# faustomorales/keras-ocr

Measured on AMD Instinct MI355X. Metric: images/sec end-to-end Pipeline.recognize() @768x768, higher is better.
Workload: dtype f32 (fp32 operands as 2 fp16 pieces [F(4,3) / head layers] or 3 bf16 pieces [1x1, dilated], 3 / 6 MFMA products, fp32 accumulate; fp32-class error vs fp64: tests/test_conv_gpu.py)

## Files before the change

keras_ocr_amd/csrc/api.cpp:

```cpp
#include "abi.h"
#include "taps.h"
#include <cmath>
#include <algorithm>
#include <mutex>
#include <set>

int arena_reserve(kocr_ctx* ctx, Arena& a, size_t bytes) {
  ctx->invalidate_results();
  a.requested = bytes;
  a.peak = 0;
  const size_t guard = a.gctx ? ARENA_GUARD_RESERVE : 0;
  if (bytes + guard <= a.cap) return KOCR_OK;
  if (a.base) {
    if (!a.guards.empty()) arena_guard_check(a);
    KOCR_HIP(ctx, hipStreamSynchronize(ctx->stream));
    KOCR_HIP(ctx, hipFree(a.base));
    a.base = nullptr;
    a.cap = 0;
  }
  const size_t want = bytes + (bytes >> 3) + 4096 + guard;
  void* p = nullptr;
  hipError_t e = hipMalloc(&p, want);
  if (e != hipSuccess) {
    ctx->set_err("workspace hipMalloc(" + std::to_string(want) + " B) failed: " + hipGetErrorString(e));
// ... 267 lines not shown
  TapsEnd taps_end{ctx, TAPS_CRNN};
  return crnn_batches(ctx, M, batch);
}

extern "C" {

int kocr_create(kocr_ctx** out, int hip_device) {
  if (!out) return KOCR_EINVAL;
  *out = nullptr;
  int count = 0;
  if (hipGetDeviceCount(&count) != hipSuccess || hip_device < 0 || hip_device >= count) return KOCR_EHIP;
  if (hipSetDevice(hip_device) != hipSuccess) return KOCR_EHIP;
  kocr_ctx* c = new kocr_ctx();
  if (const char* e = getenv("KOCR_SPLIT"))
    c->split_mode = (!strcmp(e, "f16") || !strcmp(e, "fp16") || !strcmp(e, "f16x2")) ? KOCR_SPLIT_F16X2
                    : (!strcmp(e, "f16x1") || !strcmp(e, "fast"))                     ? KOCR_SPLIT_F16X1
                                                                                      : KOCR_SPLIT_BF16X3;
  {
    auto on = [](const char* name, bool dflt) {
      const char* e = getenv(name);
      return e ? atoi(e) != 0 : dflt;
    };
    c->sw.dense_splitk = on("KOCR_DENSE_SPLITK", true);
    c->sw.lstm16 = on("KOCR_LSTM16", true);
    c->sw.hs16 = on("KOCR_HS16", true);
    c->sw.k5 = on("KOCR_K5", true);
    c->sw.up2x = on("KOCR_UP2X", true);
    c->sw.w43h = on("KOCR_W43H", true);
    c->sw.w43 = on("KOCR_W43", true);
    c->sw.w43r = on("KOCR_W43R", true);
    c->sw.w43v = on("KOCR_W43V", true);
    c->sw.w43rag = on("KOCR_W43RAG", true);
    c->sw.w43dilh = on("KOCR_W43DILH", true);
    c->sw.cells = on("KOCR_CELLS", true);
    c->sw.wsplit = on("KOCR_WSPLIT", true);
    c->sw.dsplit = on("KOCR_DSPLIT", true);
    c->sw.hsplit = on("KOCR_HSPLIT", true);
    c->sw.first = on("KOCR_FIRST", true);
  }
  c->prof_layers = getenv("KOCR_PROF_LAYERS") != nullptr;
  if (const char* e = getenv("KOCR_LINFOLD")) c->opt_linfold = atoi(e) != 0;
  if (const char* e = getenv("KOCR_UPFOLD")) c->opt_upfold = atoi(e) != 0;
  c->device = hip_device;
  if (hipDeviceGetAttribute(&c->n_cu, hipDeviceAttributeMultiprocessorCount, hip_device) != hipSuccess ||
      hipStreamCreateWithFlags(&c->own_stream, hipStreamNonBlocking) != hipSuccess) {
    delete c;
    return KOCR_EHIP;
  }
  c->stream = c->own_stream;
  *out = c;
  return KOCR_OK;
}

void kocr_destroy(kocr_ctx* ctx) {
  if (!ctx) return;
  hipSetDevice(ctx->device);
  hipStreamSynchronize(ctx->stream);
  craft_free(ctx);
  crnn_free(ctx);
  for (void* p : ctx->owned) hipFree(p);
  for (Arena* a : {&ctx->ws, &ctx->pp, &ctx->pp2, &ctx->io, &ctx->pl, &ctx->bx, &ctx->chw, &ctx->chr})
    if (a->base) hipFree(a->base);
  for (auto& pd : ctx->pending) {
    hipEventDestroy(pd.a);
    hipEventDestroy(pd.b);
  }
// ... 1145 lines not shown
```

keras_ocr_amd/csrc/common.h:

```cpp
#pragma once
#include <hip/hip_runtime.h>
#include <stdint.h>
#include <string>
#include <vector>
#include <map>
#include <atomic>
#include <cstdio>
#include <cstring>
#include <type_traits>
#include "../../include/kocr.h"

#define KOCR_HIP(ctx, expr)                                                         \
  do {                                                                              \
    hipError_t _e = (expr);                                                         \
    if (_e != hipSuccess) {                                                         \
      (ctx)->set_err(std::string(#expr) + ": " + hipGetErrorString(_e) + " at " +   \
                     __FILE__ + ":" + std::to_string(__LINE__));                    \
      return KOCR_EHIP;                                                             \
    }                                                                               \
  } while (0)

#define KOCR_TRY(expr)            \
  do {                            \
    int _rc = (expr);             \
// ... 113 lines not shown
    return c;
  }
};

struct PatternTables {
  const int* hdr = nullptr;
  const int2* nodes = nullptr;
  const int2* states = nullptr;
  const int* pred = nullptr;
};

struct kocr_ctx {
  int device = 0;
  hipStream_t own_stream = nullptr;
  hipStream_t stream = nullptr;
  std::string err;
  void set_err(const std::string& s) { err = s; }

  int split_mode = KOCR_SPLIT_F16X2;
  bool opt_linfold = true, opt_upfold = true;
  int min_area_rect = KOCR_RECT_EXACT;
  struct Switches {
    bool dense_splitk = true;
    bool lstm16 = true;
    bool hs16 = true;
    bool k5 = true;
    bool up2x = true;
    bool w43h = true;
    bool w43 = true;
    bool w43r = true;
    bool w43v = true;
    bool w43rag = true;
    bool w43dilh = true;
    bool cells = true;
    bool wsplit = true;
    bool dsplit = true;
    bool hsplit = true;
    bool first = true;
  } sw;
  bool prof_layers = false;
  int n_cu = 0;

  unsigned* d_amax = nullptr;
  int amax_used = 0;
  static constexpr int AMAX_SLOTS = 1 << 16;
  int amax_begin();
  unsigned* amax_slots(int n);

  Arena ws, pp, pp2, io, pl;
  Arena bx;
  static constexpr int N_ARENAS = 8;
  inline Arena* arena_at(int i);
  static const char* arena_name(int i) {
    static const char* const names[N_ARENAS] = {"ws", "pp", "pp2", "io", "pl", "bx", "chw", "chr"};
    return i >= 0 && i < N_ARENAS ? names[i] : nullptr;
  }
  struct GuardDamage {
    int count = 0, arena = -1;
    size_t offset = 0, byte = 0;
  } guard_damage;
  int ws_reserve(size_t bytes);
  void ws_reset() { ws.reset(); }
  void* ws_alloc(size_t bytes);

  std::vector<void*> owned;
  int dev_alloc(void** out, size_t bytes);
// ... 510 lines not shown
```

keras_ocr_amd/csrc/conv_w43.hip:

```cpp
#include "w43_common.h"
#include <utility>


template <int POOL, int DBG = 0, int DIL = 0>
__global__ __launch_bounds__(256) void conv_w43_kernel(W4Params p) {
  extern __shared__ __attribute__((aligned(16))) unsigned short As[];
  const int tid = threadIdx.x, lane = tid & 63;
  const int wn = __builtin_amdgcn_readfirstlane(tid >> 6);
  const int l31 = lane & 31, l5 = lane >> 5;
  const int nblk_n = p.Cout_pad >> 7;
  const int total = p.total_tiles;
  const int ns = p.nsteps;
  const int G = gridDim.x;
  constexpr unsigned OOB = 0x80000000u;

  const int qi = tid >> 2, q4 = tid & 3;
  const int ldst = ((qi >> 5) * 2 + (q4 >> 1)) * KH_STRIDE + ((((qi & 31) * 8) ^ ((q4 >> 1) * 32)) + (q4 & 1) * 4);
  struct Geo {
    unsigned goff[6];
    int gy;
    bool gok;
    const float* base;
  };
  auto make_geo = [&](int L, Geo& g) __attribute__((always_inline)) {
// ... 599 lines not shown
  extern __shared__ __attribute__((aligned(16))) unsigned short As[];
  const int tid = threadIdx.x, lane = tid & 63;
  const int wave = __builtin_amdgcn_readfirstlane(tid >> 6);
  const int wn = wave & 1, ph = wave >> 1;
  const int l31 = lane & 31, l5 = lane >> 5;
  const int total = p.total_tiles;
  const int ncg = p.Cin >> 4;
  const int G = gridDim.x;
  constexpr unsigned OOB = 0x80000000u;

  auto tile_mt = [&](int mp, int m) {
    if constexpr (GEO) {
      const int rq = (int)w4_fdiv((unsigned)mp, p.dv_tpr), cb = mp - rq * p.tiles_per_row;
      return (2 * rq + m) * p.tiles_per_row + cb;
    } else {
      return 2 * mp + m;
    }
  };

  const int q4 = tid & 3, qd0 = (tid >> 2) & (QPR - 1), r0 = GEO ? (tid >> 6) : (tid >> 7);
  const int cp = tid & 7, qd1 = GEO ? ((tid >> 3) & 15) : qd0, r1 = GEO ? 4 + (tid >> 7) : r0 + 2;
  int ldst[2];
  ldst[0] = r0 * ROW_STRIDE + (q4 >> 1) * KHS + (((qd0 * 8) ^ ((q4 >> 1) * 32)) + (q4 & 1) * 4);
  if constexpr (GEO)
    ldst[1] = r1 * ROW_STRIDE + (cp >> 2) * KHS + (((qd1 * 8) ^ ((cp >> 2) * 32)) + (cp & 3) * 2);
  else
    ldst[1] = r1 * ROW_STRIDE + (q4 >> 1) * KHS + (((qd1 * 8) ^ ((q4 >> 1) * 32)) + (q4 & 1) * 4);
  struct Geo {
    unsigned off0[2];
    unsigned ok;
    const float* base;
  };
  auto make_geo = [&](int L, Geo& g, bool& left, bool& right) __attribute__((always_inline)) {
    const int mp = kocr_xcd_remap(L < total ? L : 0, total);
    int y0, x0;
    const long pm = w4_mtile_pm0<1>(p, tile_mt(mp, 0), y0, x0);
    g.base = p.in + (pm * p.in_cs + p.in_co) - (long)(p.W + 1) * p.in_cs;
    g.off0[0] = (unsigned)(((r0 * p.W + 4 * qd0) * p.in_cs + q4 * 4) * 4);
    g.off0[1] = (unsigned)(((r1 * p.W + 4 * qd1) * p.in_cs + (GEO ? cp * 2 : q4 * 4)) * 4);
    g.ok = ((L < total && (unsigned)(y0 - 1 + r0) < (unsigned)p.H) ? 1u : 0u) |
           ((L < total && (unsigned)(y0 - 1 + r1) < (unsigned)p.H) ? 2u : 0u);
    left = x0 == 0;
    right = x0 + TCOLS >= p.W;
  };
  Geo gc, gn;
  bool lc, rc, ln, rn;
  int ld_cg = 0;
  bool ld_next = false;
  typedef typename std::conditional<GEO != 0, v2f, v4f>::type raw1_t;
  auto load_item0 = [&](v4f (&raw)[6]) __attribute__((always_inline)) {
    const int soff = ld_cg * 64;
    const bool ok = (ld_next ? gn.ok : gc.ok) & 1u;
    const unsigned off0 = (ld_next ? gn.off0[0] : gc.off0[0]) | (ok ? 0u : OOB);
    const bool left = (ld_next ? ln : lc) && qd0 == 0, right = (ld_next ? rn : rc) && qd0 == QPR - 1;
    const unsigned stride = (unsigned)(p.in_cs * 4);
    const __amdgpu_buffer_rsrc_t rsrc = w4_rsrc(ld_next ? gn.base : gc.base, 0x80000000u);
#pragma unroll
    for (int k = 0; k < 6; ++k) {
      const unsigned padk = (k == 0 ? (left ? OOB : 0u) : 0u) | (k == 5 ? (right ? OOB : 0u) : 0u);
      raw[k] = __builtin_bit_cast(v4f, __builtin_amdgcn_raw_buffer_load_b128(rsrc, (off0 + k * stride) | padk, soff, 0));
    }
  };
  auto load_item1 = [&](raw1_t (&raw)[6]) __attribute__((always_inline)) {
    const int soff = ld_cg * 64;
    const bool ok = ((ld_next ? gn.ok : gc.ok) >> 1) & 1u;
    const unsigned off0 = (ld_next ? gn.off0[1] : gc.off0[1]) | (ok ? 0u : OOB);
    const bool left = (ld_next ? ln : lc) && qd1 == 0, right = (ld_next ? rn : rc) && qd1 == QPR - 1;
// ... 91 lines not shown
        mfma12(cur, pp);
      }
      __builtin_amdgcn_sched_barrier(0);
      {
        int sn = s0 + ky + 1;
        sn = sn >= ns ? sn - ns : sn;
        w4_load_w(bw[pp], w_ptr + (size_t)sn * w_step, 3 * ph + pp);
      }
      if (g == 3) load_item0(raw0);
    }
    load_item1(raw1);
    advance();
  };

  make_geo(blockIdx.x, gc, lc, rc);
  make_geo(blockIdx.x + G, gn, ln, rn);
  load_item0(raw0);
  load_item1(raw1);
  advance();
#pragma unroll
  for (int pl = 0; pl < 3; ++pl) w4_load_w(bw[pl], w_ptr, 3 * ph + pl);
#pragma unroll
  for (int xi = 0; xi < 6; ++xi) {
    produce4(raw0, As, xi, 0);
    produce_item1(As, xi);
  }
  load_item0(raw0);
  load_item1(raw1);
  advance();
  __syncthreads();
  load_a(a0, As, 0, 0);

  for (int L = blockIdx.x; L < total; L += G) {
    const int mp = kocr_xcd_remap(L, total);
#pragma unroll
    for (int x = 0; x < 3; ++x)
#pragma unroll
      for (int m = 0; m < 2; ++m)
#pragma unroll
        for (int r = 0; r < 16; ++r) acc[x][m][r] = 0.f;
    __builtin_amdgcn_s_waitcnt(0x0F70);
    for (int cg = 0; cg < ncg; cg += 2) {
      phase(As, As + BUF_R, 3 * cg, 0);
      phase(As + BUF_R, As, 3 * cg + 3, 1);
    }
    gc = gn;
    lc = ln;
    rc = rn;
    make_geo(L + 2 * G, gn, ln, rn);
    ld_next = false;

    {
      const int n = wn * 32 + l31;
      const int nc = n < p.Cout ? n : p.Cout - 1;
      const float pa = p.pre_a[nc], pb = p.pre_b[nc];
      const bool has_post = p.post_a != nullptr;
      const float qa = has_post ? p.post_a[nc] : 1.f, qb = has_post ? p.post_b[nc] : 0.f;
      const bool live = n < p.Cout;
      const float lo = p.relu ? 0.f : -INFINITY;
      auto act = [&](float v) { return fmaxf(v * pa + pb, lo); };
      v4f* xch = reinterpret_cast<v4f*>(As + BUF_R);
      float out[4][16];
      auto halves = [&](auto ph_c) __attribute__((always_inline)) {
        constexpr int PH = decltype(ph_c)::value;
        auto partial = [&](auto m_c, int r, float (&o)[4]) __attribute__((always_inline)) {
          constexpr int M = decltype(m_c)::value;
          const float u = acc[0][M][r], v = acc[1][M][r], w = acc[2][M][r];
// ... 113 lines not shown
    if constexpr (GEO == 2)
      return ((w >> 1) * 2 + kh) * 128 + (w & 1) * 64 + ((q * 8) ^ (kh * 32));
    else
      return w * ROW_STRIDE + kh * KHS + ((q * 8) ^ (kh * 32));
  };
  auto tile_org = [&](int mp, int& y0, int& x0) -> long {
    if constexpr (GEO == 2) {
      const int rq = (int)w4_fdiv((unsigned)mp, p.dv_tpr), cb = mp - rq * p.tiles_per_row;
      const int ho = p.H >> 3;
      const int nimg = (int)w4_fdiv((unsigned)rq, p.dv_hh), ro = rq - nimg * ho;
      y0 = 8 * ro;
      x0 = 32 * cb;
      return ((long)nimg * p.H + y0) * p.W + x0;
    } else {
      const int rq = (int)w4_fdiv((unsigned)mp, p.dv_tpr), cb = mp - rq * p.tiles_per_row;
      return w4_mtile_pm0<1>(p, 2 * rq * p.tiles_per_row + cb, y0, x0);
    }
  };

  const int q4 = tid & 3, qd0 = (tid >> 2) & (QPR - 1), r0 = GEO == 2 ? (tid >> 5) : (tid >> 6);
  const int cp = tid & 7;
  const int qd1 = GEO == 2 ? ((tid >> 3) & 7) : ((tid >> 3) & 15);
  const int r1 = GEO == 2 ? 8 + ((tid >> 6) & 1) : 4 + (tid >> 7);
  int ldst[2];
  ldst[0] = slot(r0, q4 >> 1, qd0) + (q4 & 1) * 4;
  ldst[1] = slot(r1, cp >> 2, qd1) + (cp & 3) * 2;
  struct Geo {
    unsigned off0[2];
    unsigned ok;
    const float* base;
  };
  auto make_geo = [&](int L, Geo& g, bool& left, bool& right) __attribute__((always_inline)) {
    int mp, nt_unused;
    w4_decode(p, kocr_xcd_remap(L < total ? L : 0, total), nblk_n, mp, nt_unused);
    int y0, x0;
    const long pm = tile_org(mp, y0, x0);
    g.base = p.in + (pm * p.in_cs + p.in_co) - (long)(p.W + 1) * p.in_cs;
    g.off0[0] = (unsigned)(((r0 * p.W + 4 * qd0) * p.in_cs + q4 * 4) * 4);
    g.off0[1] = (unsigned)(((r1 * p.W + 4 * qd1) * p.in_cs + cp * 2) * 4);
    g.ok = ((L < total && (unsigned)(y0 - 1 + r0) < (unsigned)p.H) ? 1u : 0u) |
           ((L < total && (unsigned)(y0 - 1 + r1) < (unsigned)p.H) ? 2u : 0u);
    left = x0 == 0;
    right = x0 + TCOLS >= p.W;
  };
  Geo gc, gn;
  bool lc, rc, ln, rn;
  int ld_cg = 0;
  bool ld_next = false;
  auto load_item0 = [&](v4f (&raw)[6]) __attribute__((always_inline)) {
    const int soff = ld_cg * 64;
    const bool ok = (ld_next ? gn.ok : gc.ok) & 1u;
    const unsigned off0 = (ld_next ? gn.off0[0] : gc.off0[0]) | (ok ? 0u : OOB);
    const bool left = (ld_next ? ln : lc) && qd0 == 0, right = (ld_next ? rn : rc) && qd0 == QPR - 1;
    const unsigned stride = (unsigned)(p.in_cs * 4);
    const __amdgpu_buffer_rsrc_t rsrc = w4_rsrc(ld_next ? gn.base : gc.base, 0x80000000u);
#pragma unroll
    for (int k = 0; k < 6; ++k) {
      const unsigned padk = (k == 0 ? (left ? OOB : 0u) : 0u) | (k == 5 ? (right ? OOB : 0u) : 0u);
      raw[k] = __builtin_bit_cast(v4f, __builtin_amdgcn_raw_buffer_load_b128(rsrc, (off0 + k * stride) | padk, soff, 0));
    }
  };
  auto load_item1 = [&](v2f (&raw)[6]) __attribute__((always_inline)) {
    const int soff = ld_cg * 64;
    const bool ok = ((ld_next ? gn.ok : gc.ok) >> 1) & 1u;
    const unsigned off0 = (ld_next ? gn.off0[1] : gc.off0[1]) | (ok ? 0u : OOB);
    const bool left = (ld_next ? ln : lc) && qd1 == 0, right = (ld_next ? rn : rc) && qd1 == QPR - 1;
    const unsigned stride = (unsigned)(p.in_cs * 4);
// ... 81 lines not shown
      mfma12(a0, 2 * q);
      interleave();
      __builtin_amdgcn_sched_barrier(0);
      load_b(2 * q);
      __builtin_amdgcn_sched_barrier(0);
      if (q < 2) {
        load_a(a0, bufc, KY, 2 * q + 2);
        produce(2 * q + 1);
        mfma12(a1, 2 * q + 1);
        interleave();
      } else if constexpr (KY < 2) {
        load_a(a0, bufc, KY + 1, 0);
        produce(5);
        mfma12(a1, 5);
        interleave();
      } else {
        __syncthreads();
        load_a(a0, bufn, 0, 0);
        __builtin_amdgcn_sched_barrier(0);
        mfma12(a1, 5);
      }
      __builtin_amdgcn_sched_barrier(0);
      load_b(2 * q + 1);
    }
  };

  make_geo(blockIdx.x, gc, lc, rc);
  make_geo(blockIdx.x + G, gn, ln, rn);
  load_item0(raw0);
  load_item1(raw1);
  advance();
  {
    int mp0, nt0;
    w4_decode(p, kocr_xcd_remap(blockIdx.x, total), nblk_n, mp0, nt0);
    const unsigned short* w0 = w_tile(nt0);
#pragma unroll
    for (int xi = 0; xi < 6; ++xi) w4_load_w(bw[xi], w0, xi);
  }
#pragma unroll
  for (int xi = 0; xi < 6; ++xi) {
    produce4(raw0, As, xi, 0);
    produce_item1(As, xi);
  }
  load_item0(raw0);
  load_item1(raw1);
  advance();
  __syncthreads();
  load_a(a0, As, 0, 0);

  for (int L = blockIdx.x; L < total; L += G) {
    int mp, nt, mp_n, nt_n;
    w4_decode(p, kocr_xcd_remap(L, total), nblk_n, mp, nt);
    w4_decode(p, kocr_xcd_remap(L + G < total ? L + G : L, total), nblk_n, mp_n, nt_n);
    const unsigned short* w_ptr = w_tile(nt);
    const unsigned short* w_after = w_tile(nt_n);
    auto w_at = [&](int s) { return s < ns ? w_ptr + (size_t)s * w_step : w_after; };
#pragma unroll
    for (int x = 0; x < 6; ++x)
#pragma unroll
      for (int m = 0; m < 2; ++m)
#pragma unroll
        for (int r = 0; r < 16; ++r) acc[x][m][r] = 0.f;
    __builtin_amdgcn_s_waitcnt(0x0F70);
    for (int cg = 0; cg < ncg; cg += 2) {
      step(std::integral_constant<int, 0>{}, As, As + BUF_R, w_at(3 * cg + 1));
      load_item0(raw0);
      step(std::integral_constant<int, 1>{}, As, As + BUF_R, w_at(3 * cg + 2));
      load_item1(raw1);
      advance();
      step(std::integral_constant<int, 2>{}, As, As + BUF_R, w_at(3 * cg + 3));
      step(std::integral_constant<int, 0>{}, As + BUF_R, As, w_at(3 * cg + 4));
      load_item0(raw0);
      step(std::integral_constant<int, 1>{}, As + BUF_R, As, w_at(3 * cg + 5));
      load_item1(raw1);
      advance();
      step(std::integral_constant<int, 2>{}, As + BUF_R, As, w_at(3 * cg + 6));
    }
    gc = gn;
    lc = ln;
    rc = rn;
    make_geo(L + 2 * G, gn, ln, rn);
    ld_next = false;

    {
      const int n = (nt * 4 + wn) * 32 + l31;
      const int nc = n < p.Cout ? n : p.Cout - 1;
// ... 316 lines not shown
      p.cellWv = in.cellWv;
      p.cells_per_row = in.W / in.cellW;
    }
  }
  w4_div_magic((unsigned)(p.qpr > 0 ? p.qpr : 1), p.dv_qpr);
  w4_div_magic((unsigned)L.dil, p.dv_dil);
  w4_div_magic((unsigned)in.H, p.dv_h);
  w4_div_magic((unsigned)(p.rq_per_img ? p.rq_per_img : 1), p.dv_rq);
  w4_div_magic((unsigned)(p.cellW ? p.cellW : 1), p.dv_wc);
  p.total_tiles = p.n_mpairs * (p.Cout_pad / (narrow ? 64 : 128));
  w4_div_magic((unsigned)p.tiles_per_row, p.dv_tpr);
  w4_div_magic((unsigned)(geo2 ? in.H / 8 : in.H / 2), p.dv_hh);
  w4_div_magic((unsigned)p.n_mpairs, p.dv_mp);
  w4_div_magic((unsigned)(in.H * in.W), p.dv_hw);
  if (q.tracks()) {
    p.amax_out = (!fuse || need_full) ? out.amax : nullptr;
    p.amax_pool = fuse ? pool->amax : nullptr;
  }
  if (q.pieces) {
    const unsigned* slots = in.amax;
    if (!slots) {
      unsigned* tmp = ctx->amax_slots(in.N);
      if (!tmp) KOCR_FAIL(ctx, KOCR_ECAPACITY, "conv " + L.name + ": out of max-|x| slots");
      KOCR_TRY(launch_absmax(ctx, in, tmp));
      slots = tmp;
    }
    p.amax_in = slots;
    if (ctx->range_on) KOCR_TRY(launch_range_stats(ctx, L.name, in, slots, 12));
    p.wgt = L.d_w4h;
    p.pre_a = L.d_pre_a_h;
  }
  w4_div_magic((unsigned)(p.Cout_pad / (narrow ? 64 : 128)), p.dv_nb);
  p.m_fastest = (size_t)L.Cin * L.w4_cout_pad * 3 * 36 > ((size_t)6 << 20) ? 1 : 0;
  std::string nm, fam;
  w43_names(ctx, L, q, nm, fam);
  kocr_note_dispatch(fam.c_str(), L, in);
  const double Malg = cells ? (double)in.N * in.cells() * (in.H - 1) * in.cellWv : (double)M;
  const double flops = 2.0 * Malg * L.Kreal * L.Cout;
  const double bytes = 4.0 * (Malg * L.Cin + Malg * L.Cout * ((fuse && !need_full) ? 0.25 : 1.0) + (double)L.Kreal * L.Cout);
  {
    ProfScope ps(ctx, nm.c_str(), flops, bytes);
#ifdef KOCR_DEV_SWITCHES
    static const int dbg = getenv("KOCR_W43_DBG") ? atoi(getenv("KOCR_W43_DBG")) : 0;
    if (dbg >= 1 && dbg <= 15 && !fuse) return w4_launch_dbg(ctx, p, dbg, std::make_integer_sequence<int, 15>{});
#endif
    switch (q.arr) {
      case 'v':
        if (q.pieces)
          KOCR_TRY(launch_w43vh(ctx, p, fuse, q.geo, q.pieces, q.mode));
        else if (q.geo == 2)
          KOCR_TRY((w4v_launch<0, 2>(ctx, p)));
        else
          KOCR_TRY((fuse ? w4v_launch<1, 1>(ctx, p) : w4v_launch<0, 1>(ctx, p)));
        break;
      case 'r':
        if (q.pieces)
          KOCR_TRY(launch_w43rh(ctx, p, fuse, q.pieces, q.mode));
        else if (q.geo == 1)
          KOCR_TRY((fuse ? w4r_launch<1, 1>(ctx, p) : w4r_launch<0, 1>(ctx, p)));
        else
          KOCR_TRY((fuse ? w4r_launch<1, 0>(ctx, p) : w4r_launch<0, 0>(ctx, p)));
        break;
      case 'f': KOCR_TRY(launch_w43fh(ctx, p, q.pieces)); break;
      case 'n': KOCR_TRY(fuse ? w4n_launch<1>(ctx, p) : w4n_launch<0>(ctx, p)); break;
      default:
        if (L.dil != 1)
// ... 13 lines not shown
```

keras_ocr_amd/csrc/conv_w43h.hip:

```cpp
#include "w43_common.h"
#include "probe_clock.h"

namespace {

#define W4H_SCALED_CONSTANTS(sc)                                                                       \
  const float k_s = (sc), k_sA = (sc) * W4_A, k_sB = (sc) * W4_B, k_sA2 = (sc) * W4_A2, k_sB2 = (sc) * W4_B2, \
              k_sA2B2 = (sc) * W4_A2B2, k_sA2PB2 = (sc) * W4_A2PB2
template <class T>
__device__ __forceinline__ T w4h_transform(const T (&d)[6], int xi, float k_s, float k_sA, float k_sB, float k_sA2, float k_sB2,
                                           float k_sA2B2, float k_sA2PB2) {
  switch (xi) {
    case 0: return (k_sA2B2 * d[0] - k_sA2PB2 * d[2]) + k_s * d[4];
    case 1: return (k_s * d[4] - k_sB2 * d[2]) + k_sA * (d[3] - W4_B2 * d[1]);
    case 2: return (k_s * d[4] - k_sB2 * d[2]) - k_sA * (d[3] - W4_B2 * d[1]);
    case 3: return (k_s * d[4] - k_sA2 * d[2]) + k_sB * (d[3] - W4_A2 * d[1]);
    case 4: return (k_s * d[4] - k_sA2 * d[2]) - k_sB * (d[3] - W4_A2 * d[1]);
    default: return (k_sA2B2 * d[1] - k_sA2PB2 * d[3]) + k_s * d[5];
  }
}

constexpr int W4H_TOP = 12;

}

// ... 37 lines not shown
      y0 = (GEO == 2 ? 8 : 4) * ro;
      x0 = TCOLS * cb;
      nimg_o = nimg;
      return ((long)nimg * p.H + y0) * p.W + x0;
    } else if constexpr (GEO == 2) {
      const int rq = (int)w4_fdiv((unsigned)mp, p.dv_tpr), cb = mp - rq * p.tiles_per_row;
      const int ho = p.H >> 3;
      const int nimg = (int)w4_fdiv((unsigned)rq, p.dv_hh), ro = rq - nimg * ho;
      y0 = 8 * ro;
      x0 = 32 * cb;
      return ((long)nimg * p.H + y0) * p.W + x0;
    } else {
      const int rq = (int)w4_fdiv((unsigned)mp, p.dv_tpr), cb = mp - rq * p.tiles_per_row;
      return w4_mtile_pm0<1>(p, 2 * rq * p.tiles_per_row + cb, y0, x0);
    }
  };

  const int q4 = tid & 3, qd0 = (tid >> 2) & (QPR - 1), r0 = GEO == 2 ? (tid >> 5) : (tid >> 6);
  const int cp = tid & 7;
  const int qd1 = GEO == 2 ? ((tid >> 3) & 7) : ((tid >> 3) & 15);
  const int r1 = GEO == 2 ? 8 + ((tid >> 6) & 1) : 4 + (tid >> 7);
  int ldst[2];
  ldst[0] = slot(r0, q4 >> 1, qd0) + (q4 & 1) * 4;
  ldst[1] = slot(r1, cp >> 2, qd1) + (cp & 3) * 2;
  struct Geo {
    unsigned off0[2];
    unsigned ok;
    int e;
    int e1, qb;
    const float* base;
  };
  auto make_geo = [&](int L, Geo& g, bool& left, bool& right) __attribute__((always_inline)) {
    int mp, nt_unused;
    w4_decode(p, kocr_xcd_remap(L < total ? L : 0, total), nblk_n, mp, nt_unused);
    int y0, x0, nimg = 0;
    const long pm = tile_org(mp, y0, x0, nimg);
    g.base = p.in + (pm * p.in_cs + p.in_co) - (long)(p.W + 1) * p.in_cs;
    const int tid = wn * 64 + kocr_fresh_lane();
    const int q4 = tid & 3, qd0 = (tid >> 2) & (QPR - 1), r0 = GEO == 2 ? (tid >> 5) : (tid >> 6);
    const int cp = tid & 7;
    const int qd1 = GEO == 2 ? ((tid >> 3) & 7) : ((tid >> 3) & 15);
    const int r1 = GEO == 2 ? 8 + ((tid >> 6) & 1) : 4 + (tid >> 7);
    g.off0[0] = (unsigned)(((r0 * p.W + 4 * qd0) * p.in_cs + q4 * 4) * 4);
    g.off0[1] = (unsigned)(((r1 * p.W + 4 * qd1) * p.in_cs + cp * 2) * 4);
    g.ok = ((L < total && (unsigned)(y0 - 1 + r0) < (unsigned)p.H) ? 1u : 0u) |
           ((L < total && (unsigned)(y0 - 1 + r1) < (unsigned)p.H) ? 2u : 0u);
    g.e1 = 0;
    g.qb = QPR;
    if constexpr (MODE == 2) {
      const int j0 = (int)w4_fdiv((unsigned)x0, p.dv_wc);
      const int j1 = j0 + 1 < p.cells_per_row ? j0 + 1 : j0;
      const int c0 = __builtin_amdgcn_readfirstlane(nimg * p.cells_per_row + j0), c1 = __builtin_amdgcn_readfirstlane(nimg * p.cells_per_row + j1);
      g.e = kocr_scale_exp_bits(kocr_sload(p.amax_in + c0), W4H_TOP);
      g.e1 = kocr_scale_exp_bits(kocr_sload(p.amax_in + c1), W4H_TOP);
      const int qb = ((j0 + 1) * p.cellW - x0) >> 2;
      g.qb = qb < QPR ? qb : QPR;
    } else if constexpr (MODE == 1) {
      g.e = kocr_scale_exp_bits(kocr_sload(p.amax_in + __builtin_amdgcn_readfirstlane(nimg)), W4H_TOP);
    } else {
      g.e = kocr_scale_exp_bits(kocr_sload(p.amax_in + __builtin_amdgcn_readfirstlane((int)w4_fdiv((unsigned)pm, p.dv_hw))), W4H_TOP);
    }
    if constexpr (MODE == 1) {
      const int c0 = x0 - 1 + 4 * qd0, c1 = x0 - 1 + 4 * qd1;
      unsigned cm = 0;
#pragma unroll
      for (int k = 0; k < 6; ++k)
        cm |= ((unsigned)(c0 + k) < (unsigned)p.W ? 0u : (4u << k)) | ((unsigned)(c1 + k) < (unsigned)p.W ? 0u : (256u << k));
// ... 190 lines not shown
      interleave();
      __builtin_amdgcn_sched_barrier(0);
      load_b(2 * q);
      __builtin_amdgcn_sched_barrier(0);
      if (q < 2) {
        load_a(a0, bufc, KY, 2 * q + 2);
        produce(2 * q + 1);
        mfma_pt(a1, bw[SLOT][2 * q + 1], 2 * q + 1);
        interleave();
      } else if constexpr (KY < 2) {
        load_a(a0, bufc, KY + 1, 0);
        produce(5);
        mfma_pt(a1, bw[SLOT][5], 5);
        interleave();
      } else {
        if constexpr (!(DBG & 32)) __syncthreads();
        load_a(a0, bufn, 0, 0);
        __builtin_amdgcn_sched_barrier(0);
        mfma_pt(a1, bw[SLOT][5], 5);
      }
      __builtin_amdgcn_sched_barrier(0);
      load_b(2 * q + 1);
    }
  };

  w4_stage_coef(p, coef, tid);
  make_geo(blockIdx.x, gc, lc, rc);
  make_geo(blockIdx.x + G, gn, ln, rn);
  load_item0(raw0);
  load_item1(raw1);
  advance();
  {
    int mp0, nt0;
    w4_decode(p, kocr_xcd_remap(blockIdx.x, total), nblk_n, mp0, nt0);
    const unsigned w0 = w_tile(nt0);
#pragma unroll
    for (int st = 0; st < 2; ++st)
#pragma unroll
      for (int xi = 0; xi < 6; ++xi)
#pragma unroll
        for (int s = 0; s < NP; ++s)
          bw[st][xi][s] = __builtin_bit_cast(hf8, __builtin_amdgcn_raw_buffer_load_b128(wrsrc, wlane, (int)(w0 + st * w_step + (unsigned)(xi * 2 + s) * 1024u), 0));
  }
#pragma unroll
  for (int xi = 0; xi < 6; ++xi) {
    produce4(raw0, As, xi, 0, kocr_pow2(gc.e), kocr_pow2(gc.e1), gc.qb);
    produce2(raw1, As, xi, kocr_pow2(gc.e), kocr_pow2(gc.e1), gc.qb);
  }
  load_item0(raw0);
  load_item1(raw1);
  advance();
  __syncthreads();
  load_a(a0, As, 0, 0);

  PROBE_RESTART();
  for (int L = blockIdx.x; L < total; L += G) {
    int mp, nt, mp_n, nt_n;
    w4_decode(p, kocr_xcd_remap(L, total), nblk_n, mp, nt);
    w4_decode(p, kocr_xcd_remap(L + G < total ? L + G : L, total), nblk_n, mp_n, nt_n);
    const unsigned w_ptr = w_tile(nt), w_after = w_tile(nt_n);
    auto w_at = [&](int s) { return s < ns ? w_ptr + (unsigned)s * w_step : w_after + (unsigned)(s - ns) * w_step; };
    const float s_cur = kocr_pow2(gc.e), s_nxt = kocr_pow2(gn.e);
    const float s_cur1 = kocr_pow2(gc.e1), s_nxt1 = kocr_pow2(gn.e1);
    const int qb_nxt = gn.qb;
    const float unscale = kocr_pow2(-gc.e);
    const float unscale1 = kocr_pow2(-gc.e1);
    const int qb_cur = gc.qb;
#pragma unroll
    for (int x = 0; x < 6; ++x)
#pragma unroll
      for (int m = 0; m < 2; ++m)
#pragma unroll
        for (int r = 0; r < 16; ++r) acc[x][m][r] = 0.f;
    PROBE_T(5);
    __builtin_amdgcn_s_waitcnt(0x0F70);
    PROBE_T(4);
    for (int cg = 0; cg < ncg; cg += 2) {
      using I0 = std::integral_constant<int, 0>;
      using I1 = std::integral_constant<int, 1>;
      using I2 = std::integral_constant<int, 2>;
      step(I0{}, I0{}, As, As + BUF_R, w_at(3 * cg + 2), s_cur, s_cur1, qb_cur);
      load_item0(raw0);
      step(I1{}, I1{}, As, As + BUF_R, w_at(3 * cg + 3), s_cur, s_cur1, qb_cur);
      load_item1(raw1);
      advance();
      step(I2{}, I0{}, As, As + BUF_R, w_at(3 * cg + 4), s_cur, s_cur1, qb_cur);
      const bool same = cg + 2 < ncg;
      const float s_odd = same ? s_cur : s_nxt, s_odd1 = same ? s_cur1 : s_nxt1;
      const int qb_odd = same ? qb_cur : qb_nxt;
      step(I0{}, I1{}, As + BUF_R, As, w_at(3 * cg + 5), s_odd, s_odd1, qb_odd);
      load_item0(raw0);
      step(I1{}, I0{}, As + BUF_R, As, w_at(3 * cg + 6), s_odd, s_odd1, qb_odd);
// ... 222 lines not shown
  constexpr unsigned OOB = 0x80000000u;

  auto tile_mt = [&](int mp, int m) {
    const int rq = (int)w4_fdiv((unsigned)mp, p.dv_tpr), cb = mp - rq * p.tiles_per_row;
    return (2 * rq + m) * p.tiles_per_row + cb;
  };
  auto mtile_org = [&](int mp, int m, int& y0, int& x0, int& nimg_o) -> long {
    if constexpr (MODE == 1) {
      const int rq = (int)w4_fdiv((unsigned)mp, p.dv_tpr), cb = mp - rq * p.tiles_per_row;
      const int nimg = (int)w4_fdiv((unsigned)rq, p.dv_rq), ro = rq - nimg * p.rq_per_img;
      y0 = 4 * ro + 2 * m;
      x0 = TCOLS * cb;
      nimg_o = nimg;
      return ((long)nimg * p.H + y0) * p.W + x0;
    } else {
      const long pm = w4_mtile_pm0<1>(p, tile_mt(mp, m), y0, x0);
      nimg_o = (int)w4_fdiv((unsigned)pm, p.dv_hw);
      return pm;
    }
  };

  const int q4 = tid & 3, qd0 = (tid >> 2) & (QPR - 1), r0 = tid >> 6;
  const int cp = tid & 7, qd1 = (tid >> 3) & 15, r1 = 4 + (tid >> 7);
  int ldst[2];
  ldst[0] = r0 * ROW_STRIDE + (q4 >> 1) * KHS + (((qd0 * 8) ^ ((q4 >> 1) * 32)) + (q4 & 1) * 4);
  ldst[1] = r1 * ROW_STRIDE + (cp >> 2) * KHS + (((qd1 * 8) ^ ((cp >> 2) * 32)) + (cp & 3) * 2);
  struct Geo {
    unsigned off0[2];
    unsigned ok;
    int e;
    const float* base;
  };
  auto make_geo = [&](int L, Geo& g, bool& left, bool& right) __attribute__((always_inline)) {
    const int mp = kocr_xcd_remap(L < total ? L : 0, total);
    int y0, x0, nimg;
    const long pm = mtile_org(mp, 0, y0, x0, nimg);
    g.base = p.in + (pm * p.in_cs + p.in_co) - (long)(p.W + 1) * p.in_cs;
    const int tid = wave * 64 + kocr_fresh_lane();
    const int q4 = tid & 3, qd0 = (tid >> 2) & (QPR - 1), r0 = tid >> 6;
    const int cp = tid & 7, qd1 = (tid >> 3) & 15, r1 = 4 + (tid >> 7);
    g.off0[0] = (unsigned)(((r0 * p.W + 4 * qd0) * p.in_cs + q4 * 4) * 4);
    g.off0[1] = (unsigned)(((r1 * p.W + 4 * qd1) * p.in_cs + cp * 2) * 4);
    g.ok = ((L < total && (unsigned)(y0 - 1 + r0) < (unsigned)p.H) ? 1u : 0u) |
           ((L < total && (unsigned)(y0 - 1 + r1) < (unsigned)p.H) ? 2u : 0u);
    g.e = kocr_scale_exp_bits(kocr_sload(p.amax_in + __builtin_amdgcn_readfirstlane(nimg)), W4H_TOP);
    if constexpr (MODE == 1) {
      const int c0 = x0 - 1 + 4 * qd0, c1 = x0 - 1 + 4 * qd1;
      unsigned cm = 0;
#pragma unroll
      for (int k = 0; k < 6; ++k)
        cm |= ((unsigned)(c0 + k) < (unsigned)p.W ? 0u : (4u << k)) | ((unsigned)(c1 + k) < (unsigned)p.W ? 0u : (256u << k));
      g.ok |= cm;
      left = right = false;
    } else {
      left = x0 == 0;
      right = x0 + TCOLS >= p.W;
    }
  };
  Geo gc, gn;
  bool lc, rc, ln, rn;
  int ld_cg = 0;
  bool ld_next = false;
  auto load_item0 = [&](v4f (&raw)[6]) __attribute__((always_inline)) {
    const int soff = ld_cg * 64;
    const unsigned okb = ld_next ? gn.ok : gc.ok;
    const bool ok = okb & 1u;
    const unsigned off0 = (ld_next ? gn.off0[0] : gc.off0[0]) | (ok ? 0u : OOB);
// ... 141 lines not shown
        for (int s = 0; s < NP; ++s)
          bw[pp][s] = __builtin_bit_cast(hf8, __builtin_amdgcn_raw_buffer_load_b128(wrsrc, wlane, (int)(wq + (unsigned)(pp * 2 + s) * 1024u), 0));
      }
      if (g == 3) load_item0(r0);
    }
    load_item1(r1);
    advance();
  };

  w4_stage_coef(p, coef, tid);
  make_geo(blockIdx.x, gc, lc, rc);
  make_geo(blockIdx.x + G, gn, ln, rn);
  load_item0(raw0[0]);
  load_item1(raw1[0]);
  advance();
#pragma unroll
  for (int g = 0; g < NBW; ++g)
#pragma unroll
    for (int s = 0; s < NP; ++s)
      bw[g][s] = __builtin_bit_cast(hf8, __builtin_amdgcn_raw_buffer_load_b128(wrsrc, wlane, (int)(w_wave + (unsigned)(g / 3) * w_step + (unsigned)((g % 3) * 2 + s) * 1024u), 0));
#pragma unroll
  for (int xi = 0; xi < 6; ++xi) {
    produce4(raw0[0], As, xi, kocr_pow2(gc.e));
    produce2(raw1[0], As, xi, kocr_pow2(gc.e));
  }
  load_item0(raw0[0]);
  load_item1(raw1[0]);
  advance();
  __syncthreads();
  load_a(a0, As, 0, 0);

  PROBE_T0();
  for (int L = blockIdx.x; L < total; L += G) {
    const int mp = kocr_xcd_remap(L, total);
    const float s_cur = kocr_pow2(gc.e), s_nxt = kocr_pow2(gn.e);
    const float unscale = kocr_pow2(-gc.e);
#pragma unroll
    for (int x = 0; x < 3; ++x)
#pragma unroll
      for (int m = 0; m < 2; ++m)
#pragma unroll
        for (int r = 0; r < 16; ++r) acc[x][m][r] = 0.f;
    PROBE_T(5);
    __builtin_amdgcn_s_waitcnt(0x0F70);
    PROBE_T(4);
    for (int cg = 0; cg < ncg; cg += 2) {
      phase(As, As + BUF_R, 3 * cg, 0, s_cur);
      phase(As + BUF_R, As, 3 * cg + 3, 1, cg + 2 < ncg ? s_cur : s_nxt);
    }

    PROBE_T(0);
    {
      const int lane_e = kocr_fresh_lane();
      const int l31e = lane_e & 31, l5e = lane_e >> 5;
      const int n = wn * 32 + l31e;
      int y0, x0, timg;
      const long pm = mtile_org(mp, ph, y0, x0, timg);
      const int nimg = __builtin_amdgcn_readfirstlane(timg);
      const unsigned seen_out = p.amax_out ? kocr_amax_peek(p.amax_out + nimg) : 0u;
      const unsigned seen_pool = p.amax_pool ? kocr_amax_peek(p.amax_pool + nimg) : 0u;
      const float pa = coef[n] * unscale, pb = coef[p.Cout_pad + n];
      const bool has_post = p.post_a != nullptr;
      const float qa = coef[2 * p.Cout_pad + n], qb = coef[3 * p.Cout_pad + n];
      const bool live = n < p.Cout;
      const float lo = p.relu ? 0.f : -INFINITY;
      auto act = [&](float v) { return fmaxf(v * pa + pb, lo); };
      v4f* xch = reinterpret_cast<v4f*>(As + BUF_R);
// ... 666 lines not shown
```

keras_ocr_amd/csrc/w43_common.h:

```cpp
#pragma once
#include "split_common.h"
#include <type_traits>
#include <cmath>
#include <algorithm>
#include <vector>

struct W4Params {
  const float* in;
  const unsigned short* wgt;
  float* out;
  const float* pre_a;
  const float* pre_b;
  const float* post_a;
  const float* post_b;
  int H, W, Cin, in_cs, in_co;
  int Cout, Cout_pad, out_cs, out_co;
  int relu;
  int nsteps;
  int Mtotal;
  int total_mtiles;
  float* pool_out;
  int pool_cs, pool_co, write_full, tiles_per_row;
  int total_tiles;
  int n_mpairs;
  int dil;
  int qpr;
  int m_fastest;
  unsigned* amax_out;
  unsigned* amax_pool;
  unsigned dv_tpr[2];
  unsigned dv_hh[2];
  unsigned dv_mp[2];
  unsigned dv_nb[2];
  unsigned dv_hw[2];
  const unsigned* amax_in;
  int Wv;
  unsigned dv_w[2];
  int rq_per_img;
  unsigned dv_rq[2];
  unsigned dv_qpr[2], dv_dil[2], dv_h[2];
  int cellW, cellWv, cells_per_row;
  unsigned dv_wc[2];
};

static inline void w4_div_magic(unsigned d, unsigned (&out)[2]) {
  if (d <= 1) {
    out[0] = 0;
    out[1] = 0;
    return;
  }
  unsigned L = 0;
  while ((1ull << L) < d) ++L;
  out[0] = (unsigned)(((1ull << 32) * ((1ull << L) - d)) / d + 1);
  out[1] = L - 1;
}

namespace {

__device__ __forceinline__ unsigned w4_fdiv(unsigned n, const unsigned (&dv)[2]) {
  if (dv[0] == 0 && dv[1] == 0) return n;
  const unsigned t = __umulhi(n, dv[0]);
  return (t + ((n - t) >> 1)) >> dv[1];
}

constexpr double W4_PA = 0.625, W4_PB = 1.5;
constexpr float W4_A = (float)W4_PA, W4_B = (float)W4_PB;
constexpr float W4_A2 = (float)(W4_PA * W4_PA), W4_B2 = (float)(W4_PB * W4_PB);
constexpr float W4_A3 = (float)(W4_PA * W4_PA * W4_PA), W4_B3 = (float)(W4_PB * W4_PB * W4_PB);
constexpr float W4_A2B2 = (float)(W4_PA * W4_PA * W4_PB * W4_PB), W4_A2PB2 = (float)(W4_PA * W4_PA + W4_PB * W4_PB);

constexpr int KH_STRIDE = 256;
constexpr int PLANE = 2 * 2 * KH_STRIDE;
constexpr int BUF = 6 * 3 * PLANE;
constexpr int LDS_BYTES = 2 * BUF * 2;

template <int POOL>
__device__ __forceinline__ long w4_mtile_pm0(const W4Params& p, int mt, int& y0, int& x0) {
  if constexpr (POOL) {
    const int rp_lin = (int)w4_fdiv((unsigned)mt, p.dv_tpr), cb = mt - rp_lin * p.tiles_per_row;
    const int hh = p.H >> 1;
    const int nimg = (int)w4_fdiv((unsigned)rp_lin, p.dv_hh), rp = rp_lin - nimg * hh;
    y0 = 2 * rp;
    x0 = cb * 64;
    return ((long)nimg * p.H + y0) * p.W + x0;
  } else {
    y0 = x0 = 0;
    return (long)mt * 128;
  }
}

__device__ __forceinline__ void w4_decode(const W4Params& p, int tile, int nblk_n, int& mp, int& nt) {
  const bool mf = p.m_fastest != 0;
  const unsigned dv[2] = {mf ? p.dv_mp[0] : p.dv_nb[0], mf ? p.dv_mp[1] : p.dv_nb[1]};
  const int quot = (int)w4_fdiv((unsigned)tile, dv);
  const int rem = tile - quot * (mf ? p.n_mpairs : nblk_n);
  nt = mf ? quot : rem;
  mp = mf ? rem : quot;
}

__device__ __forceinline__ void w4_stage_coef(const W4Params& p, float* coef, int tid) {
  for (int i = tid; i < p.Cout_pad; i += 256) {
    const int c = i < p.Cout ? i : p.Cout - 1;
    coef[i] = p.pre_a[c];
    coef[p.Cout_pad + i] = p.pre_b[c];
    coef[2 * p.Cout_pad + i] = p.post_a ? p.post_a[c] : 1.f;
    coef[3 * p.Cout_pad + i] = p.post_a ? p.post_b[c] : 0.f;
  }
}
constexpr int W4_COEF_BYTES_MAX = 4 * 1024 * 4;

__device__ __forceinline__ __amdgpu_buffer_rsrc_t w4_rsrc(const float* base, unsigned bytes) {
  const unsigned long long bb = (unsigned long long)base;
  const unsigned long long bbu = ((unsigned long long)(unsigned)__builtin_amdgcn_readfirstlane((int)(bb >> 32)) << 32) |
                                 (unsigned)__builtin_amdgcn_readfirstlane((int)bb);
  return __builtin_amdgcn_make_buffer_rsrc((void*)bbu, 0, (int)__builtin_amdgcn_readfirstlane((int)bytes), 0x00020000);
}

}

template <class T>
__device__ __forceinline__ T w4_transform(const T (&d)[6], int xi) {
  switch (xi) {
    case 0: return (W4_A2B2 * d[0] - W4_A2PB2 * d[2]) + d[4];
    case 1: return (d[4] - W4_B2 * d[2]) + W4_A * (d[3] - W4_B2 * d[1]);
    case 2: return (d[4] - W4_B2 * d[2]) - W4_A * (d[3] - W4_B2 * d[1]);
    case 3: return (d[4] - W4_A2 * d[2]) + W4_B * (d[3] - W4_A2 * d[1]);
    case 4: return (d[4] - W4_A2 * d[2]) - W4_B * (d[3] - W4_A2 * d[1]);
    default: return (W4_A2B2 * d[1] - W4_A2PB2 * d[3]) + d[5];
  }
}
// ... 60 lines not shown
```

Measured before the change: 260.2.

## Walk Winograd conv tiles in column strips for better cache locality

Adds a tile-order remapping that visits output M-tiles in vertical strips of a few tiles wide instead of row-major across the full image, applied in the w43 and w43h persistent conv kernels. The aim is to keep neighbouring tiles that share halo input rows resident in L2/MALL across concurrently running workgroups. The remap costs a few magic-number divisions per tile, with parameters read from kernarg memory. Strip width defaults to 8 or 16 tiles and can be overridden with an env var.

```diff
diff --git a/keras_ocr_amd/csrc/api.cpp b/keras_ocr_amd/csrc/api.cpp
--- a/keras_ocr_amd/csrc/api.cpp
+++ b/keras_ocr_amd/csrc/api.cpp
@@ -323,6 +323,7 @@
     c->sw.w43v = on("KOCR_W43V", true);
     c->sw.w43rag = on("KOCR_W43RAG", true);
     c->sw.w43dilh = on("KOCR_W43DILH", true);
+    if (const char* e = getenv("KOCR_W43_ORDER")) c->sw.w43strips = !strcmp(e, "rows") ? 0 : atoi(e) > 0 ? atoi(e) : -1;
     c->sw.cells = on("KOCR_CELLS", true);
     c->sw.wsplit = on("KOCR_WSPLIT", true);
     c->sw.dsplit = on("KOCR_DSPLIT", true);
diff --git a/keras_ocr_amd/csrc/common.h b/keras_ocr_amd/csrc/common.h
--- a/keras_ocr_amd/csrc/common.h
+++ b/keras_ocr_amd/csrc/common.h
@@ -169,6 +169,7 @@
     bool w43v = true;
     bool w43rag = true;
     bool w43dilh = true;
+    int w43strips = -1;
     bool cells = true;
     bool wsplit = true;
     bool dsplit = true;
diff --git a/keras_ocr_amd/csrc/conv_w43.hip b/keras_ocr_amd/csrc/conv_w43.hip
--- a/keras_ocr_amd/csrc/conv_w43.hip
+++ b/keras_ocr_amd/csrc/conv_w43.hip
@@ -655,7 +655,7 @@
     const float* base;
   };
   auto make_geo = [&](int L, Geo& g, bool& left, bool& right) __attribute__((always_inline)) {
-    const int mp = kocr_xcd_remap(L < total ? L : 0, total);
+    const int mp = w4_walk(p, kocr_xcd_remap(L < total ? L : 0, total));
     int y0, x0;
     const long pm = w4_mtile_pm0<1>(p, tile_mt(mp, 0), y0, x0);
     g.base = p.in + (pm * p.in_cs + p.in_co) - (long)(p.W + 1) * p.in_cs;
@@ -813,7 +813,7 @@
   load_a(a0, As, 0, 0);
 
   for (int L = blockIdx.x; L < total; L += G) {
-    const int mp = kocr_xcd_remap(L, total);
+    const int mp = w4_walk(p, kocr_xcd_remap(L, total));
 #pragma unroll
     for (int x = 0; x < 3; ++x)
 #pragma unroll
@@ -993,7 +993,7 @@
   };
   auto make_geo = [&](int L, Geo& g, bool& left, bool& right) __attribute__((always_inline)) {
     int mp, nt_unused;
-    w4_decode(p, kocr_xcd_remap(L < total ? L : 0, total), nblk_n, mp, nt_unused);
+    w4_decode2(p, kocr_xcd_remap(L < total ? L : 0, total), nblk_n, mp, nt_unused);
     int y0, x0;
     const long pm = tile_org(mp, y0, x0);
     g.base = p.in + (pm * p.in_cs + p.in_co) - (long)(p.W + 1) * p.in_cs;
@@ -1141,7 +1141,7 @@
   advance();
   {
     int mp0, nt0;
-    w4_decode(p, kocr_xcd_remap(blockIdx.x, total), nblk_n, mp0, nt0);
+    w4_decode2(p, kocr_xcd_remap(blockIdx.x, total), nblk_n, mp0, nt0);
     const unsigned short* w0 = w_tile(nt0);
 #pragma unroll
     for (int xi = 0; xi < 6; ++xi) w4_load_w(bw[xi], w0, xi);
@@ -1159,8 +1159,8 @@
 
   for (int L = blockIdx.x; L < total; L += G) {
     int mp, nt, mp_n, nt_n;
-    w4_decode(p, kocr_xcd_remap(L, total), nblk_n, mp, nt);
-    w4_decode(p, kocr_xcd_remap(L + G < total ? L + G : L, total), nblk_n, mp_n, nt_n);
+    w4_decode2(p, kocr_xcd_remap(L, total), nblk_n, mp, nt);
+    w4_decode2(p, kocr_xcd_remap(L + G < total ? L + G : L, total), nblk_n, mp_n, nt_n);
     const unsigned short* w_ptr = w_tile(nt);
     const unsigned short* w_after = w_tile(nt_n);
     auto w_at = [&](int s) { return s < ns ? w_ptr + (size_t)s * w_step : w_after; };
@@ -1543,6 +1543,10 @@
   }
   w4_div_magic((unsigned)(p.Cout_pad / (narrow ? 64 : 128)), p.dv_nb);
   p.m_fastest = (size_t)L.Cin * L.w4_cout_pad * 3 * 36 > ((size_t)6 << 20) ? 1 : 0;
+  const bool grid2d = q.arr == 'v' || (q.arr == 'r' && (q.pieces || q.geo == 1));
+  const int sw_ord = ctx->sw.w43strips;
+  const int strip = !grid2d ? 0 : sw_ord < 0 ? tile_order_strip_width(p.tiles_per_row, geo2 ? 32 : 64) : sw_ord;
+  p.ord = tile_order_make(p.tiles_per_row, p.tiles_per_row > 0 ? p.n_mpairs / p.tiles_per_row : 0, strip);
   std::string nm, fam;
   w43_names(ctx, L, q, nm, fam);
   kocr_note_dispatch(fam.c_str(), L, in);
diff --git a/keras_ocr_amd/csrc/conv_w43h.hip b/keras_ocr_amd/csrc/conv_w43h.hip
--- a/keras_ocr_amd/csrc/conv_w43h.hip
+++ b/keras_ocr_amd/csrc/conv_w43h.hip
@@ -93,7 +93,7 @@
   };
   auto make_geo = [&](int L, Geo& g, bool& left, bool& right) __attribute__((always_inline)) {
     int mp, nt_unused;
-    w4_decode(p, kocr_xcd_remap(L < total ? L : 0, total), nblk_n, mp, nt_unused);
+    w4_decode2(p, kocr_xcd_remap(L < total ? L : 0, total), nblk_n, mp, nt_unused);
     int y0, x0, nimg = 0;
     const long pm = tile_org(mp, y0, x0, nimg);
     g.base = p.in + (pm * p.in_cs + p.in_co) - (long)(p.W + 1) * p.in_cs;
@@ -350,7 +350,7 @@
   advance();
   {
     int mp0, nt0;
-    w4_decode(p, kocr_xcd_remap(blockIdx.x, total), nblk_n, mp0, nt0);
+    w4_decode2(p, kocr_xcd_remap(blockIdx.x, total), nblk_n, mp0, nt0);
     const unsigned w0 = w_tile(nt0);
 #pragma unroll
     for (int st = 0; st < 2; ++st)
@@ -374,8 +374,8 @@
   PROBE_RESTART();
   for (int L = blockIdx.x; L < total; L += G) {
     int mp, nt, mp_n, nt_n;
-    w4_decode(p, kocr_xcd_remap(L, total), nblk_n, mp, nt);
-    w4_decode(p, kocr_xcd_remap(L + G < total ? L + G : L, total), nblk_n, mp_n, nt_n);
+    w4_decode2(p, kocr_xcd_remap(L, total), nblk_n, mp, nt);
+    w4_decode2(p, kocr_xcd_remap(L + G < total ? L + G : L, total), nblk_n, mp_n, nt_n);
     const unsigned w_ptr = w_tile(nt), w_after = w_tile(nt_n);
     auto w_at = [&](int s) { return s < ns ? w_ptr + (unsigned)s * w_step : w_after + (unsigned)(s - ns) * w_step; };
     const float s_cur = kocr_pow2(gc.e), s_nxt = kocr_pow2(gn.e);
@@ -664,7 +664,7 @@
     const float* base;
   };
   auto make_geo = [&](int L, Geo& g, bool& left, bool& right) __attribute__((always_inline)) {
-    const int mp = kocr_xcd_remap(L < total ? L : 0, total);
+    const int mp = w4_walk(p, kocr_xcd_remap(L < total ? L : 0, total));
     int y0, x0, nimg;
     const long pm = mtile_org(mp, 0, y0, x0, nimg);
     g.base = p.in + (pm * p.in_cs + p.in_co) - (long)(p.W + 1) * p.in_cs;
@@ -872,7 +872,7 @@
 
   PROBE_T0();
   for (int L = blockIdx.x; L < total; L += G) {
-    const int mp = kocr_xcd_remap(L, total);
+    const int mp = w4_walk(p, kocr_xcd_remap(L, total));
     const float s_cur = kocr_pow2(gc.e), s_nxt = kocr_pow2(gn.e);
     const float unscale = kocr_pow2(-gc.e);
 #pragma unroll
diff --git a/keras_ocr_amd/csrc/tile_order.h b/keras_ocr_amd/csrc/tile_order.h
--- /dev/null
+++ b/keras_ocr_amd/csrc/tile_order.h
@@ -0,0 +1,64 @@
+#pragma once
+
+#if defined(__HIPCC__)
+#define KOCR_TO_HD __host__ __device__ __forceinline__
+#else
+#define KOCR_TO_HD inline
+#endif
+
+static inline void w4_div_magic(unsigned d, unsigned (&out)[2]) {
+  if (d <= 1) {
+    out[0] = 0;
+    out[1] = 0;
+    return;
+  }
+  unsigned L = 0;
+  while ((1ull << L) < d) ++L;
+  out[0] = (unsigned)(((1ull << 32) * ((1ull << L) - d)) / d + 1);
+  out[1] = L - 1;
+}
+
+KOCR_TO_HD unsigned tile_order_div(unsigned n, unsigned mul, unsigned sh) {
+  const unsigned t = (unsigned)(((unsigned long long)n * mul) >> 32);
+  return (mul | sh) ? (t + ((n - t) >> 1)) >> sh : n;
+}
+
+struct TileOrder {
+  unsigned bits;
+  unsigned strip_tiles;
+  unsigned mul_strip, mul_rem;
+};
+
+static inline TileOrder tile_order_make(int tpr, int rows, int pc) {
+  TileOrder o;
+  int lg = 0;
+  while (lg < 5 && (1 << (lg + 1)) <= pc) ++lg;
+  const bool strips = pc >= 1 && pc < tpr && rows > 0 && tpr / (1 << lg) < (1 << 14);
+  const unsigned w = 1u << lg, rem = strips ? (unsigned)tpr % w : 0u;
+  unsigned ds[2], dr[2];
+  o.strip_tiles = strips ? (unsigned)rows * w : 1u;
+  w4_div_magic(o.strip_tiles, ds);
+  w4_div_magic(rem > 0 ? rem : 1u, dr);
+  o.mul_strip = ds[0];
+  o.mul_rem = dr[0];
+  o.bits = strips ? ((unsigned)lg | rem << 3 | ds[1] << 8 | dr[1] << 13 | ((unsigned)tpr / w) << 18) : 0u;
+  return o;
+}
+
+KOCR_TO_HD int tile_order_index(unsigned bits, unsigned strip_tiles, unsigned mul_strip, unsigned mul_rem, int tpr, int j) {
+  const unsigned lg = bits & 7u, rem = (bits >> 3) & 31u, nfull = bits >> 18;
+  const unsigned strip = tile_order_div((unsigned)j, mul_strip, (bits >> 8) & 31u);
+  const bool last = strip >= nfull;
+  const unsigned jj = (unsigned)j - strip * strip_tiles;
+  const unsigned rq = last ? tile_order_div(jj, mul_rem, (bits >> 13) & 31u) : jj >> lg;
+  const unsigned mp = rq * (unsigned)tpr + (strip << lg) + (jj - rq * (last ? rem : 1u << lg));
+  return bits ? (int)mp : j;
+}
+KOCR_TO_HD int tile_order_mp(const TileOrder& o, int tpr, int j) {
+  return tile_order_index(o.bits, o.strip_tiles, o.mul_strip, o.mul_rem, tpr, j);
+}
+
+static inline int tile_order_strip_width(int tiles_per_row, int tile_cols) {
+  const int pc = tile_cols >= 64 ? 8 : 16;
+  return tiles_per_row < pc ? tiles_per_row : pc;
+}
diff --git a/keras_ocr_amd/csrc/w43_common.h b/keras_ocr_amd/csrc/w43_common.h
--- a/keras_ocr_amd/csrc/w43_common.h
+++ b/keras_ocr_amd/csrc/w43_common.h
@@ -1,5 +1,7 @@
 #pragma once
 #include "split_common.h"
+#include "tile_order.h"
+#include <cstddef>
 #include <type_traits>
 #include <cmath>
 #include <algorithm>
@@ -41,19 +43,8 @@
   unsigned dv_qpr[2], dv_dil[2], dv_h[2];
   int cellW, cellWv, cells_per_row;
   unsigned dv_wc[2];
+  TileOrder ord;
 };
-
-static inline void w4_div_magic(unsigned d, unsigned (&out)[2]) {
-  if (d <= 1) {
-    out[0] = 0;
-    out[1] = 0;
-    return;
-  }
-  unsigned L = 0;
-  while ((1ull << L) < d) ++L;
-  out[0] = (unsigned)(((1ull << 32) * ((1ull << L) - d)) / d + 1);
-  out[1] = L - 1;
-}
 
 namespace {
 
@@ -96,6 +87,23 @@
   const int rem = tile - quot * (mf ? p.n_mpairs : nblk_n);
   nt = mf ? quot : rem;
   mp = mf ? rem : quot;
+}
+
+__device__ __forceinline__ int w4_walk(const W4Params& p, int j) {
+#if defined(__HIP_DEVICE_COMPILE__)
+  typedef const unsigned __attribute__((address_space(4))) cu4;
+  typedef const char __attribute__((address_space(4))) cc4;
+  unsigned off = (unsigned)offsetof(W4Params, ord);
+  asm volatile("" : "+s"(off));
+  cu4* q = (cu4*)((cc4*)__builtin_amdgcn_kernarg_segment_ptr() + off);
+  return tile_order_index(q[0], q[1], q[2], q[3], p.tiles_per_row, j);
+#else
+  return tile_order_mp(p.ord, p.tiles_per_row, j);
+#endif
+}
+__device__ __forceinline__ void w4_decode2(const W4Params& p, int tile, int nblk_n, int& mp, int& nt) {
+  w4_decode(p, tile, nblk_n, mp, nt);
+  mp = w4_walk(p, mp);
 }
 
 __device__ __forceinline__ void w4_stage_coef(const W4Params& p, float* coef, int tid) {
```

Result: no change. 260.7, median of 6 (+0.2%).
